# pengzhangzhi/ab_opt

Hardware: AMD Instinct MI355X
Metric: denoising steps/sec (256-res complex, 100-step sampler) (higher is better)
Workload: dtype f32

## Files before the change

ab_opt_amd/csrc/ipa_core.hip:

```cpp
#include <cstdlib>
#include <type_traits>
#include "tail_common.h"
#include "node_task.h"
#include "kernels.h"

namespace abopt {

constexpr int NPW = 8, RPW = BI / NPW;
constexpr int NTH = 1024;
constexpr int SROW = 16 * JC + 4;
constexpr int SCLD = 17;
constexpr float kLog2e = 1.4426950408889634f;
constexpr float kSqrt13 = 0.5773502691896258f;
constexpr float kScale2 = kSqrt13 * kLog2e;
constexpr float kMask2 = 1e5f * kLog2e;

__device__ __forceinline__ int sp_off(int h, int kq) { return h * JC + 4 * ((kq + (h >> 1)) & 3); }

__device__ __forceinline__ void point_local(float dx, float dy, float dz, float r0, float r1, float r2, float r3, float r4, float r5, float r6, float r7,
                                            float r8, float& lx, float& ly, float& lz, float& d, float& inv) {
    lx = __builtin_fmaf(r6, dz, __builtin_fmaf(r3, dy, r0 * dx));
    ly = __builtin_fmaf(r7, dz, __builtin_fmaf(r4, dy, r1 * dx));
    lz = __builtin_fmaf(r8, dz, __builtin_fmaf(r5, dy, r2 * dx));
    d = sqrtf(__builtin_fmaf(lz, lz, __builtin_fmaf(ly, ly, lx * lx)));
// ... 683 lines not shown

constexpr int NPW2 = 4, RPW2 = BI2 / NPW2, NTH2 = 512, HPW = 6;

#define C32_L2(x, r) __builtin_fmaf((x), kScale2, mterm_[r])
__device__ long long g_clock_probe[2];
constexpr int PROF_SLOTS = 2048;
__device__ unsigned long long g_prof_span[PROF_SLOTS][2];
__global__ void prof_span_reset_kernel() {
    const int i = blockIdx.x * 256 + threadIdx.x;
    if (i < PROF_SLOTS) { g_prof_span[i][0] = ~0ull; g_prof_span[i][1] = 0ull; }
}
struct TailArgs {
    const float *wot, *wmf, *x, *ubias, *g1, *be1, *b0, *b1, *b2, *g2, *be2;
    float* out;
    unsigned* xt;
};
template <bool NF, bool QR = false, bool QC = false> struct TailArgsT : TailArgs {};
template <> struct TailArgsT<true, false, false> : TailArgs { NodeCarryArgs nc; };
template <> struct TailArgsT<false, true, false> : TailArgs { const uint8_t* qrows; };
template <> struct TailArgsT<false, true, true> : TailArgs { const int32_t* qlist; };
struct GatherRows {
    const int32_t* ql; int64_t rowbase; int L;
    __device__ __forceinline__ int at(int il) const { const int r = il < 16 ? ql[il & 15] : -1; return (unsigned)r < (unsigned)L ? r : -1; }
    __device__ __forceinline__ int64_t load(int rl) const { return rowbase + max(at(rl), 0); }
    __device__ __forceinline__ int64_t store(int rl) const { const int r = at(rl); return r < 0 ? (int64_t)-1 : rowbase + r; }
};
constexpr int C32_LOOP_LDS_FLOATS = 3 * 32 * SROW + 2 * 32 * SCLD + 32 * SCLD + 32 * 32;
__host__ __device__ constexpr size_t core32_lds_bytes(int nchunk) { return sizeof(float) * C32_LOOP_LDS_FLOATS + (size_t)nchunk * JC; }
constexpr int C32F_PTS_OFF = ((C32_LOOP_LDS_FLOATS * 4 + 2048 + 255) / 256) * 256;
constexpr int C32F_PTSLD = H * P * 3 + 4;
constexpr int C32F_LDS_BYTES = C32F_PTS_OFF + 32 * C32F_PTSLD * 4;
constexpr int C32F_U_OFF = 0, C32F_YS_OFF = MR * XLD * 4, C32F_APA_OFF = 2 * MR * XLD * 4;
constexpr int C32F_BIAS_OFF = 2 * OT_STAGE;
static_assert(2 * OT_STAGE <= 3 * 32 * SROW * 4, "staging buffers must fit into the S/P tile");
static_assert(C32F_BIAS_OFF + 3 * F * 4 <= 3 * 32 * SROW * 4 && C32F_APA_OFF + OT_NT * AP_PLANE <= 2 * OT_STAGE && OT_NT * AP_PLANE <= 32 * C32F_PTSLD * 4, "phase-2 buffers of the fused tail");
static_assert(C32F_LDS_BYTES <= 160 * 1024, "LDS of the fused block kernel");

__device__ __forceinline__ float mul_rn(float a, float b) {
#pragma clang fp contract(off)
    return a * b;
}
__device__ __forceinline__ void stage_put4(char* buf, int row, int col, float v0, float v1, float v2, float v3) {
    unsigned h0, l0, h1, l1;
    split_pair2(v0, v1, h0, l0);
    split_pair2(v2, v3, h1, l1);
    char* d = buf + row * OT_SROW + col * 2;
    *reinterpret_cast<uint2*>(d) = make_uint2(h0, h1);
    *reinterpret_cast<uint2*>(d + OT_PLANE) = make_uint2(l0, l1);
}

constexpr int NF_CARRY_WD = 9;
static_assert(2 * H == 3 * (NTH2 / 64), "three (head, half) tasks per wave");
static_assert(MR * NF_XLDS_STRIDE * 4 <= MR * XLD * 4, "the x-term tile takes the place of the u tile");
__device__ __forceinline__ void node_carry_phase(NfLdsTerms xt, NodeCarryArgs nc, const float* __restrict__ R, const float* __restrict__ t, int L, int nchunk,
                                                           int n, int ib, int tid) {
    const int lane = tid & 63, fm = lane & 15, kq = lane >> 4;
    const int wave = __builtin_amdgcn_readfirstlane(tid >> 6);
    const int tile0 = n * nchunk + 2 * ib, tiles_end = (n + 1) * nchunk;
    const float winv = nc.w_node_frag[(int64_t)H * NF_HEAD_VEC * 4 + 1];
#pragma unroll 1
    for (int k = 0; k < 3; ++k) {
        const int h = __builtin_amdgcn_readfirstlane((wave >> 1) + 4 * k);
        const float sc = nc.spatial_coef[h];
        const float gamma = (sc > 20.f) ? sc : log1pf(expf(sc));
        const float ch_ = (-1.f * gamma * 0.16666666666666666f) / 2.f;
        const float m2c = -2.f * ch_;
        const u32x4* wg = reinterpret_cast<const u32x4*>(nc.w_node_frag) + (int64_t)h * NF_HEAD_VEC + (wave & 1) * NF_LDS_VEC;
        if (wave & 1) nf_task<1, NfX::LdsTerms, NF_CARRY_WD>(nullptr, xt, wg, R, t, nc.qfrag, nc.kvfrag, L, nchunk, tiles_end, tile0, h, ch_, m2c, winv, lane, fm, kq, nc.qk_terms, ib * BI2);
        else          nf_task<0, NfX::LdsTerms, NF_CARRY_WD>(nullptr, xt, wg, R, t, nc.qfrag, nc.kvfrag, L, nchunk, tiles_end, tile0, h, ch_, m2c, winv, lane, fm, kq, nc.qk_terms, ib * BI2);
    }
}

template <bool FUSE, bool ZT, bool NF = false, bool QROWS = false, bool QC = false>
__global__ __launch_bounds__(NTH2) void ipa_core32_kernel(const float* __restrict__ qfrag, const float* __restrict__ kvfrag, const float* __restrict__ z,
                                                          const uint8_t* __restrict__ mask, const float* __restrict__ R, const float* __restrict__ t,
                                                          float* __restrict__ feat, const float* __restrict__ pbc, int L, int nib2, int xcd_remap, int z_shared,
                                                          TailArgsT<NF, QROWS, QC> ta, int prof_slot, const float* __restrict__ zt, const float* __restrict__ zsc) {
    static_assert(FUSE || !NF, "the carried projections follow the fused tail");
    static_assert(!QROWS || (FUSE && !NF), "query rows are masked in the block nobody follows");
    static_assert(!QC || QROWS, "gathered rows are masked rows");
    constexpr int NRT = QC ? 1 : 2;
    extern __shared__ __attribute__((aligned(16))) char smem_raw[];
    float* sp = reinterpret_cast<float*>(smem_raw);
    float* scl = sp + 3 * BI2 * SROW;
    float* lsum = scl + 2 * BI2 * SCLD;
    float* mlr = lsum + BI2 * SCLD;
    uint8_t* mk = reinterpret_cast<uint8_t*>(mlr + BI2 * 32);
    int n, ib;
    {
        const int b = blockIdx.x;
        if (xcd_remap == 2) {
            const int xcd = b & 7, k = b >> 3, per = nib2 * z_shared, r = k % per;
            ib = r / z_shared; n = (xcd + 8 * (k / per)) * z_shared + r % z_shared;
        } else if (xcd_remap) { const int xcd = b & 7, k = b >> 3; n = xcd + 8 * (k / nib2); ib = k % nib2; }
        else { n = b / nib2; ib = b % nib2; }
    }
    const int tid = threadIdx.x, lane = tid & 63, fm = lane & 15, kq = lane >> 4;
    const int wave = __builtin_amdgcn_readfirstlane(tid >> 6);
    const int nchunk = (L + JC - 1) / JC, nib16 = (L + BI - 1) / BI;
    const long long probe_c0 = clock64(), probe_w0 = wall_clock64();
    if (prof_slot >= 0 && threadIdx.x == 0) atomicMin(&g_prof_span[prof_slot][0], (unsigned long long)probe_w0);
    const int i0 = ib * BI2;
    const int64_t rowbase = (int64_t)n * L;
    const int64_t zbase = z_shared ? (int64_t)(n / z_shared) * L : rowbase;
    GatherRows qg_{nullptr, rowbase, L};
    if constexpr (QC) qg_.ql = ta.qlist + ((int64_t)n * nib16 + ib) * 16;
    auto fill_mask = [&]() { for (int e = tid; e < nchunk * JC; e += NTH2) mk[e] = (e < L) ? mask[rowbase + e] : 0; };
    char* const stage = smem_raw;
    float* const ptsf = reinterpret_cast<float*>(smem_raw + C32F_PTS_OFF);
    const int64_t row0f = rowbase + i0, row_endf = rowbase + L;
    TailP2Pre<NTH2 / 64> pre;
    constexpr int RD = 12;
    struct WT { u32x4 h, l; };
    auto consumer = [&](int cb, WT (&wt)[RD]) {
        const u32x4* wfr = reinterpret_cast<const u32x4*>(ta.wot) + (int64_t)cb * OT_ST * OT_WVEC + lane;
        auto kstep = [&](int i) { return min(ot_chunk_at(min(i / OT_SPC, OT_NCH - 1)) * OT_SPC + (i % OT_SPC), OT_ST - 1); };
        f32x16 acc[4];
#pragma unroll
        for (int g = 0; g < 4; ++g) acc_zero(acc[g]);
        __syncthreads();
        const char* xrd = stage + (lane & 31) * OT_SROW + (lane >> 5) * 16;
#define C32F_KSTEP(P_, KK, NK)                                                                                           \
        {                                                                                                                \
// ... 336 lines not shown
            P2H_CHUNK(0, ch)
            if (ch + 1 < nchunk) P2H_CHUNK(1, ch + 1)
        }
        } else {
        for (; ch + 3 <= nchunk; ch += 3) { P2_CHUNK(0, ch) P2_CHUNK(1, ch + 1) P2_CHUNK(2, ch + 2) }
        if (ch < nchunk) {
            P2_CHUNK(0, ch)
            if (ch + 1 < nchunk) P2_CHUNK(1, ch + 1)
        }
        }
#undef P2H_CHUNK
#undef P2H_POS
#undef P2H_POS_LAST
#undef P2H_MF
#undef P2H_SM
#undef P2H_SPLIT
#undef P2_CHUNK
#undef P2_SLOT
#undef P2_POS
#undef P2_POS_LAST
#undef P2_MF
#undef P2_SM
#undef P2_ISSUE_Z
#undef P2_ISSUE_B
#undef P2_ZRS
#undef P2_BRS
#undef P2_RSRC
#undef P2_QNEED_FENCE
#undef P2_KOFF
#undef P2_BOFF
        if constexpr (!FUSE) {
#pragma unroll
        for (int ii = 0; ii < RPW2; ++ii) {
            const int il = il0 + ii, i = i0 + il;
            const float l_fin = mlw[ii * 32 + 1];
            if (kq == 0) lsum[il * SCLD + fm] = l_fin;
            if (i < L && fm < H) {
                const bool mi = mk[i] != 0;
                const float inv = mi ? 1.f / l_fin : 0.f;
                float* fo = feat + (rowbase + i) * FEAT + fm * C + kq * 16;
#pragma unroll
                for (int r = 0; r < 4; ++r) {
                    if constexpr (ZT) {
                        const f32x4 zs = *reinterpret_cast<const f32x4*>(zsc + (zbase + i) * C + kq * 16 + r * 4);
                        reinterpret_cast<f32x4*>(fo)[r] = (f32x4){mul_rn(accP[ii][0][r], inv * zs[0]), mul_rn(accP[ii][1][r], inv * zs[1]), mul_rn(accP[ii][2][r], inv * zs[2]), mul_rn(accP[ii][3][r], inv * zs[3])};
                    } else
                    reinterpret_cast<f32x4*>(fo)[r] = (f32x4){accP[ii][0][r] * inv, accP[ii][1][r] * inv, accP[ii][2][r] * inv, accP[ii][3][r] * inv};
                }
            }
        }
        __syncthreads();
        __syncthreads();
        } else {
#pragma unroll
        for (int ii = 0; ii < RPW2; ++ii)
            if (kq == 0) lsum[(il0 + ii) * SCLD + fm] = mlw[ii * 32 + 1];
        __syncthreads();
        float rinv[RPW2];
#pragma unroll
        for (int ii = 0; ii < RPW2; ++ii) {
            bool mi;
            if constexpr (QC) mi = qr_[ii] >= 0 && mk[max(qr_[ii], 0)] != 0;
            else { const int i = i0 + il0 + ii; mi = (i < L) && mk[min(i, L - 1)] != 0; }
            rinv[ii] = mi ? 1.f / mlw[ii * 32 + 1] : 0.f;
        }
        const int ptid = wave * 64 + lane, prow = ptid >> 3, psub = ptid & 7;
        float rr_[9], tt_[3];
        {
            int64_t grow;
            if constexpr (QC) grow = qg_.load(prow); else grow = rowbase + min(i0 + prow, L - 1);
#pragma unroll
            for (int q = 0; q < 9; ++q) rr_[q] = R[grow * 9 + q];
#pragma unroll
            for (int q = 0; q < 3; ++q) tt_[q] = t[grow * 3 + q];
        }
        __syncthreads();
        auto local_of = [&](int pt, float& lx, float& ly, float& lz, float& d, float& inv) {
            const float* a = ptsf + prow * C32F_PTSLD + pt * 3;
            point_local(a[0] - tt_[0], a[1] - tt_[1], a[2] - tt_[2], rr_[0], rr_[1], rr_[2], rr_[3], rr_[4], rr_[5], rr_[6], rr_[7], rr_[8], lx, ly, lz, d, inv);
        };
        auto put_points = [&](char* buf, int col0, int pt0, int npt, bool dir) {
            float v[24];
#pragma unroll
            for (int k = 0; k < 8; ++k) {
                if (k < npt) {
                    float lx, ly, lz, d, inv;
                    local_of(pt0 + k, lx, ly, lz, d, inv);
                    v[3 * k] = dir ? mul_rn(lx, inv) : lx; v[3 * k + 1] = dir ? mul_rn(ly, inv) : ly; v[3 * k + 2] = dir ? mul_rn(lz, inv) : lz;
                }
            }
#pragma unroll
            for (int q = 0; q < 6; ++q)
                if (4 * q < 3 * npt) stage_put4(buf, prow, col0 + 4 * q, v[4 * q], v[4 * q + 1], v[4 * q + 2], v[4 * q + 3]);
        };
#pragma unroll
        for (int p = 0; p < OT_NCH; ++p) {
            if (p >= 1 && p + 1 < OT_NCH) {
                char* buf = stage + ((p + 1) & 1) * OT_STAGE;
                const int c = ot_chunk_at(p + 1);
                if (c < 4) {
                    if (fm < H) {
#pragma unroll
                        for (int ii = 0; ii < RPW2; ++ii) {
                            if constexpr (ZT) {
                                int zr_;
                                if constexpr (QC) zr_ = max(qr_[ii], 0); else zr_ = min(i0 + il0 + ii, L - 1);
                                const f32x4 zs = *reinterpret_cast<const f32x4*>(zsc + (zbase + zr_) * C + kq * 16 + c * 4);
                                stage_put4(buf, il0 + ii, fm * 16 + kq * 4, mul_rn(accP[ii][0][c], rinv[ii] * zs[0]), mul_rn(accP[ii][1][c], rinv[ii] * zs[1]),
                                           mul_rn(accP[ii][2][c], rinv[ii] * zs[2]), mul_rn(accP[ii][3][c], rinv[ii] * zs[3]));
                            } else
                            stage_put4(buf, il0 + ii, fm * 16 + kq * 4, mul_rn(accP[ii][0][c], rinv[ii]), mul_rn(accP[ii][1][c], rinv[ii]),
                                       mul_rn(accP[ii][2][c], rinv[ii]), mul_rn(accP[ii][3][c], rinv[ii]));
                        }
                    }
                } else if (c == 6) {
                    put_points(buf, psub * 24, psub * 8, 8, false);
                } else if (c == 7) {
                    put_points(buf, psub * 12, 64 + psub * 4, 4, false);
                    float dd[12];
#pragma unroll
                    for (int k = 0; k < 12; ++k) { float lx, ly, lz, inv; local_of(psub * 12 + k, lx, ly, lz, dd[k], inv); }
#pragma unroll
                    for (int q = 0; q < 3; ++q) stage_put4(buf, prow, 96 + psub * 12 + 4 * q, dd[4 * q], dd[4 * q + 1], dd[4 * q + 2], dd[4 * q + 3]);
                } else if (c == 8) {
                    put_points(buf, psub * 24, psub * 8, 8, true);
                } else {
                    put_points(buf, psub * 12, 64 + psub * 4, 4, true);
                }
            }
            __syncthreads();
        }
        }
    } else if (wave < NPW2 + 2) {
        const int h0 = (wave - NPW2) * HPW;
        const f32x4* kvn = reinterpret_cast<const f32x4*>(kvfrag) + (int64_t)n * nchunk * H * 512;
        f32x4 qr[HPW][NRT][4];
        const int qrow_ = QC ? max(qg_.at(fm), 0) : 0;
#pragma unroll
        for (int hh = 0; hh < HPW; ++hh)
#pragma unroll
            for (int rt = 0; rt < NRT; ++rt) {
                const f32x4* qg;
                if constexpr (QC) qg = reinterpret_cast<const f32x4*>(qfrag) + (((int64_t)n * nib16 + (qrow_ >> 4)) * H + h0 + hh) * (4 * 64) + kq * 16 + (qrow_ & 15);
                else qg = reinterpret_cast<const f32x4*>(qfrag) + (((int64_t)n * nib16 + min(2 * ib + rt, nib16 - 1)) * H + h0 + hh) * (4 * 64) + lane;
#pragma unroll
                for (int s_ = 0; s_ < 4; ++s_) qr[hh][rt][s_] = qg[s_ * 64];
            }
        f32x4 kf[2][4];
#define A2_ISSUE(B, HH, CH) { const f32x4* fr_ = kvn + ((int64_t)min((CH), nchunk - 1) * H + h0 + (HH)) * 512 + lane;   \
        _Pragma("unroll") for (int s_ = 0; s_ < 4; ++s_) kf[B][s_] = fr_[s_ * 64]; }
        auto produce = [&](int c, int buf) {
#pragma unroll
            for (int hh = 0; hh < HPW; ++hh) {
                const int h = h0 + hh;
                if (hh + 1 < HPW) { if (hh & 1) A2_ISSUE(0, hh + 1, c) else A2_ISSUE(1, hh + 1, c) } else A2_ISSUE(0, 0, c + 1)
#pragma unroll
                for (int rt = 0; rt < NRT; ++rt) {
                    const f32x4 q0 = qr[hh][rt][0], q1 = qr[hh][rt][1], q2 = qr[hh][rt][2], q3 = qr[hh][rt][3];
                    f32x4 acc0 = (f32x4){0.f, 0.f, 0.f, 0.f}, acc1 = acc0;
                    if constexpr (ZT) {
                        const u32x4 kh = __builtin_bit_cast(u32x4, kf[hh & 1][0]), kl = __builtin_bit_cast(u32x4, kf[hh & 1][1]);
                        const u32x4 qh = __builtin_bit_cast(u32x4, q0), ql = __builtin_bit_cast(u32x4, q1);
                        acc0 = mfma_h(kl, qh, acc0); acc0 = mfma_h(kh, ql, acc0);
#pragma unroll
                        for (int s = 0; s < 4; ++s) { acc1 = mfma4(kf[hh & 1][2][s], q2[s], acc1); if (s == 1) acc0 = mfma_h(kh, qh, acc0); }
#pragma unroll
                        for (int s = 0; s < 3; ++s) acc1 = mfma4(kf[hh & 1][3][s], q3[s], acc1);
                    }
                    else {
#pragma unroll
                    for (int s = 0; s < 4; ++s) { acc0 = mfma4(kf[hh & 1][0][s], q0[s], acc0); acc1 = mfma4(kf[hh & 1][2][s], q2[s], acc1); }
#pragma unroll
                    for (int s = 0; s < 4; ++s) { acc0 = mfma4(kf[hh & 1][1][s], q1[s], acc0); if (s < 3) acc1 = mfma4(kf[hh & 1][3][s], q3[s], acc1); }
                    }
                    const f32x4 sres = acc0 + acc1;
                    *reinterpret_cast<f32x4*>(sp + (buf * BI2 + rt * 16 + fm) * SROW + sp_off(h, kq)) = sres;
                }
                __builtin_amdgcn_sched_barrier(0);
            }
        };
        A2_ISSUE(0, 0, 0)
        fill_mask();
        __syncthreads();
        produce(0, 0);
        __syncthreads();
        int buf = 1;
        for (int c = 1; c < nchunk; ++c) {
            produce(c, buf);
            buf = (buf == 2) ? 0 : buf + 1;
            __syncthreads();
        }
        __syncthreads();
        if constexpr (!FUSE) {
        __syncthreads();
        __syncthreads();
        } else {
        WT raw[RD];
        consumer_prefetch(wave - NPW2, raw);
        __syncthreads();
        tail_p2_stage_bias(reinterpret_cast<float (*)[F]>(smem_raw + C32F_BIAS_OFF), ta.b0, ta.b1, ta.b2, tid - NPW2 * 64);
        consumer(wave - NPW2, raw);
        }
#undef A2_ISSUE
    } else {
        const int h0 = (wave - NPW2 - 2) * HPW;
        const f32x4* kvn = reinterpret_cast<const f32x4*>(kvfrag) + (int64_t)n * nchunk * H * 512;
        f32x4 vf[2][4];
        f32x4 accV[HPW][2][2], accT[HPW][2][2];
#pragma unroll
        for (int hh = 0; hh < HPW; ++hh)
#pragma unroll
            for (int rt = 0; rt < 2; ++rt)
#pragma unroll
                for (int k = 0; k < 2; ++k) { accV[hh][rt][k] = (f32x4){0.f, 0.f, 0.f, 0.f}; accT[hh][rt][k] = (f32x4){0.f, 0.f, 0.f, 0.f}; }
#define C2_ISSUE(B, HH, CH) { const f32x4* fr_ = kvn + ((int64_t)min((CH), nchunk - 1) * H + h0 + (HH)) * 512 + 4 * 64 + lane; \
        _Pragma("unroll") for (int s_ = 0; s_ < 4; ++s_) vf[B][s_] = fr_[s_ * 64]; }
        auto consume = [&](int c, int buf) {
            const int par = c & 1;
#pragma unroll
            for (int hh = 0; hh < HPW; ++hh) {
                const int h = h0 + hh;
                if (hh + 1 < HPW) { if (hh & 1) C2_ISSUE(0, hh + 1, c) else C2_ISSUE(1, hh + 1, c) } else C2_ISSUE(0, 0, c + 1)
#pragma unroll
                for (int rt = 0; rt < NRT; ++rt) {
                    const float sc = scl[(par * BI2 + rt * 16 + fm) * SCLD + h];
                    const f32x4 pa = *reinterpret_cast<const f32x4*>(sp + (buf * BI2 + rt * 16 + fm) * SROW + sp_off(h, kq));
                    if (!(FUSE && __builtin_amdgcn_ballot_w64(sc != 1.f) == 0ull)) { accV[hh][rt][0] *= sc; accV[hh][rt][1] *= sc; accT[hh][rt][0] *= sc; accT[hh][rt][1] *= sc; }
#pragma unroll
                    for (int s = 0; s < 4; ++s) {
                        accV[hh][rt][0] = mfma4(vf[hh & 1][s][0], pa[s], accV[hh][rt][0]);
                        accV[hh][rt][1] = mfma4(vf[hh & 1][s][1], pa[s], accV[hh][rt][1]);
                        accT[hh][rt][0] = mfma4(vf[hh & 1][s][2], pa[s], accT[hh][rt][0]);
                        accT[hh][rt][1] = mfma4(vf[hh & 1][s][3], pa[s], accT[hh][rt][1]);
                    }
                }
                __builtin_amdgcn_sched_barrier(0);
            }
        };
        C2_ISSUE(0, 0, 0)
        fill_mask();
        __syncthreads();
        __syncthreads();
        __syncthreads();
        int buf = 0;
        for (int c = 1; c < nchunk; ++c) {
            consume(c - 1, buf);
            buf = (buf == 2) ? 0 : buf + 1;
            __syncthreads();
        }
        consume(nchunk - 1, buf);
        WT raw[RD];
        __syncthreads();
        float* pts = FUSE ? ptsf : sp;
        char* nbuf = stage + (wave - NPW2 - 2) * OT_STAGE;
#pragma unroll
        for (int hh = 0; hh < HPW; ++hh) {
            const int h = h0 + hh;
#pragma unroll
            for (int rt = 0; rt < 2; ++rt) {
                const int il = rt * 16 + fm, i = i0 + il;
                bool mi;
                if constexpr (QC) { const int qi = rt == 0 ? qg_.at(fm) : -1; mi = qi >= 0 && mk[max(qi, 0)] != 0; }
                else mi = (i < L) && mk[min(i, L - 1)] != 0;
                const float inv = mi ? 1.f / lsum[il * SCLD + h] : 0.f;
                if constexpr (FUSE) {
                    const f32x4 a0 = accV[hh][rt][0], a1 = accV[hh][rt][1];
                    stage_put4(nbuf, il, hh * D + kq * 4, mul_rn(a0[0], inv), mul_rn(a0[1], inv), mul_rn(a0[2], inv), mul_rn(a0[3], inv));
                    stage_put4(nbuf, il, hh * D + 16 + kq * 4, mul_rn(a1[0], inv), mul_rn(a1[1], inv), mul_rn(a1[2], inv), mul_rn(a1[3], inv));
                } else if (i < L) {
                    float* fo = feat + (rowbase + i) * FEAT + H * C + h * D + kq * 4;
                    *reinterpret_cast<f32x4*>(fo) = accV[hh][rt][0] * inv;
                    *reinterpret_cast<f32x4*>(fo + 16) = accV[hh][rt][1] * inv;
                }
                float* po = pts + il * (FUSE ? C32F_PTSLD : H * P * 3) + h * (P * 3) + kq * 3;
#pragma unroll
                for (int r = 0; r < 3; ++r) { po[r] = accT[hh][rt][0][r] * inv; po[12 + r] = accT[hh][rt][1][r] * inv; }
            }
        }
        if constexpr (FUSE) {
            consumer_prefetch(wave - NPW2, raw);
            consumer(wave - NPW2, raw);
        }
        else __syncthreads();
#undef C2_ISSUE
    }
    if constexpr (!FUSE) {
        persist_point_epilogue(sp, R, t, feat, rowbase, i0, L, tid, NTH2, BI2);
    } else {
        const int64_t row0 = row0f, row_end = row_endf;
        if constexpr (QC) pre = tail_p2_prefetch<NTH2 / 64>(ta.x, ta.ubias, mask, ta.g1, ta.be1, ta.wmf, row0, row_end, wave, lane, qg_);
        else pre = tail_p2_prefetch<NTH2 / 64>(ta.x, ta.ubias, mask, ta.g1, ta.be1, ta.wmf, row0, row_end, wave, lane);
        float (*bias)[F] = reinterpret_cast<float (*)[F]>(smem_raw + C32F_BIAS_OFF);
        __syncthreads();
        const float (*us)[XLD] = reinterpret_cast<const float (*)[XLD]>(smem_raw + C32F_U_OFF);
        auto get_u = [&](int rl) { return *reinterpret_cast<const float2*>(&us[rl][2 * lane]); };
        if constexpr (QC)
        tail_p2_run<NTH2 / 64, false>(pre, get_u, reinterpret_cast<float (*)[XLD]>(smem_raw + C32F_YS_OFF), bias, smem_raw + C32F_APA_OFF,
                                      smem_raw + C32F_PTS_OFF, ta.wmf, ta.g2, ta.be2, ta.out, nullptr, 0, row0, row_end, wave, lane, ta.xt, nullptr, 0, qg_);
        else
        tail_p2_run<NTH2 / 64, false>(pre, get_u, reinterpret_cast<float (*)[XLD]>(smem_raw + C32F_YS_OFF), bias, smem_raw + C32F_APA_OFF,
                                      smem_raw + C32F_PTS_OFF, ta.wmf, ta.g2, ta.be2, ta.out, nullptr, 0, row0, row_end, wave, lane, ta.xt,
                                      NF ? reinterpret_cast<unsigned*>(smem_raw + C32F_U_OFF) : nullptr, NF_XLDS_STRIDE);
        if constexpr (NF) {
            __syncthreads();
            node_carry_phase((NfLdsTerms)(smem_raw + C32F_U_OFF), ta.nc, R, t, L, nchunk, n, ib, tid);
        }
    }
    if (blockIdx.x == 0 && tid == 0) { g_clock_probe[0] = clock64() - probe_c0; g_clock_probe[1] = wall_clock64() - probe_w0; }
    if (prof_slot >= 0 && tid == 0) atomicMax(&g_prof_span[prof_slot][1], (unsigned long long)wall_clock64());
}

struct WbList { const float* w[8]; };

__global__ __launch_bounds__(256) void pair_bias_cache_kernel(const float* __restrict__ z, WbList wl, int num_layers, float* __restrict__ cache,
                                                              int64_t rows, int L, int nchunk) {
    __shared__ __attribute__((aligned(16))) float zst[4][JC][ZSLD];
    const int wave = threadIdx.x >> 6, lane = threadIdx.x & 63, fm = lane & 15, kq = lane >> 4;
    const int64_t unit = (int64_t)blockIdx.x * 4 + wave;
    if (unit >= rows * 4) return;
    const int64_t row = unit >> 2;
    const int q0 = (int)(unit & 3);
    if (q0 >= nchunk) return;
    const float* zi = z + (row * (int64_t)L) * C;
    f32x4 wv[6][4];
#pragma unroll
    for (int l = 0; l < 6; ++l)
#pragma unroll
        for (int q = 0; q < 4; ++q) wv[l][q] = (l < num_layers && fm < H) ? reinterpret_cast<const f32x4*>(wl.w[l] + fm * C + kq * 16)[q] : (f32x4){0.f, 0.f, 0.f, 0.f};
    f32x4 zn[4];
#pragma unroll
    for (int r = 0; r < 4; ++r) zn[r] = *(reinterpret_cast<const f32x4*>(zi + (int64_t)min(q0 * JC + kq * 4 + r, L - 1) * C) + fm);
    for (int ch = q0; ch < nchunk; ch += 4) {
        wave_lds_sync();
#pragma unroll
        for (int r = 0; r < 4; ++r) *reinterpret_cast<f32x4*>(&zst[wave][kq * 4 + r][fm * 4]) = zn[r];
        if (ch + 4 < nchunk) {
#pragma unroll
            for (int r = 0; r < 4; ++r) zn[r] = *(reinterpret_cast<const f32x4*>(zi + (int64_t)min((ch + 4) * JC + kq * 4 + r, L - 1) * C) + fm);
        }
        wave_lds_sync();
        f32x4 za[4];
#pragma unroll
        for (int q = 0; q < 4; ++q) za[q] = *reinterpret_cast<const f32x4*>(&zst[wave][fm][kq * 16 + q * 4]);
        const int64_t u = (int64_t)ch * rows + row;
        auto layer = [&](int l, const f32x4 (&w4)[4]) {
            f32x4 acc4[4];
#pragma unroll
            for (int q = 0; q < 4; ++q) {
                acc4[q] = mfma4(za[q][0], w4[q][0], (f32x4){0.f, 0.f, 0.f, 0.f});
                acc4[q] = mfma4(za[q][1], w4[q][1], acc4[q]); acc4[q] = mfma4(za[q][2], w4[q][2], acc4[q]); acc4[q] = mfma4(za[q][3], w4[q][3], acc4[q]);
            }
            const f32x4 acc = (acc4[0] + acc4[1]) + (acc4[2] + acc4[3]);
            if (fm < H) *reinterpret_cast<f32x4*>(cache + ((int64_t)l * rows * nchunk + u) * (H * JC) + fm * JC + kq * 4) = acc;
        };
#pragma unroll
        for (int l = 0; l < 6; ++l)
            if (l < num_layers) layer(l, wv[l]);
        for (int l = 6; l < num_layers; ++l) {
// ... 275 lines not shown
```

ab_opt_amd/csrc/node_task.h:

```cpp
#pragma once
#include "ipa_common.h"

namespace abopt {

constexpr int NF_F = 128;
constexpr int NF_TILES = 12, NF_HT = NF_TILES / 2, NF_WAVES = 4;
constexpr int NF_KS = NF_F / 32, NF_SPL = 2;
constexpr int NF_HEAD_VEC = NF_TILES * NF_KS * NF_SPL * 64;
constexpr int NF_LDS_VEC = NF_HEAD_VEC / 2;

__device__ __forceinline__ float quad_bcast0(float v) { return __uint_as_float(__builtin_amdgcn_update_dpp(0u, __float_as_uint(v), 0x00, 0xf, 0xf, false)); }
__device__ __forceinline__ float quad_bcast1(float v) { return __uint_as_float(__builtin_amdgcn_update_dpp(0u, __float_as_uint(v), 0x55, 0xf, 0xf, false)); }
__device__ __forceinline__ float quad_bcast2(float v) { return __uint_as_float(__builtin_amdgcn_update_dpp(0u, __float_as_uint(v), 0xAA, 0xf, 0xf, false)); }

enum class NfX { GlobalF32, GlobalTerms, LdsTerms };
constexpr int NF_XLDS_STRIDE = NF_F + 4;
typedef const __attribute__((address_space(3))) unsigned* NfLdsTerms;
typedef const __attribute__((address_space(3))) u32x4* NfLdsVec;
__device__ __forceinline__ float nf_mul_rn(float a, float b) {
#pragma clang fp contract(off)
    return a * b;
}
template <int HALF, NfX XS, int WD, class XP, class WP>
__device__ __forceinline__ void nf_task(const float* __restrict__ x, XP xt, WP wl, const float* __restrict__ R, const float* __restrict__ t,
                                        float* __restrict__ qfrag, float* __restrict__ kvfrag, int L, int nchunk, int total_tiles, int tile0, int h,
                                        float ch_, float m2c, float winv, int lane, int fm, int kq, int qk_terms, int xrow0 = 0) {
    constexpr bool XT = XS != NfX::GlobalF32;
    constexpr int XLD_ = XS == NfX::LdsTerms ? NF_XLDS_STRIDE : NF_F;
    int64_t rowbase[2], row[2];
    int cbs[2];
#pragma unroll
    for (int rt = 0; rt < 2; ++rt) {
        const int tile = min(tile0 + rt, total_tiles - 1);
        const int n = tile / nchunk;
        cbs[rt] = tile % nchunk;
        rowbase[rt] = (int64_t)n * L;
        row[rt] = rowbase[rt] + min(cbs[rt] * JC + fm, L - 1);
    }
    auto xvec = [&](int rt, int word) {
        if constexpr (XS == NfX::LdsTerms) return *reinterpret_cast<NfLdsVec>(xt + (min(cbs[rt] * JC + fm, L - 1) - xrow0) * XLD_ + word);
        else return *reinterpret_cast<const u32x4*>(xt + row[rt] * XLD_ + word);
    };
    f32x4 xa[2][2];
    Split2 xn[2];
#pragma unroll
    for (int rt = 0; rt < 2; ++rt) {
        if constexpr (XT) {
            xn[rt].h = xvec(rt, kq * 4);
            xn[rt].l = xvec(rt, 64 + kq * 4);
        } else {
            xa[rt][0] = *reinterpret_cast<const f32x4*>(x + row[rt] * NF_F + kq * 8);
            xa[rt][1] = *reinterpret_cast<const f32x4*>(x + row[rt] * NF_F + kq * 8 + 4);
        }
    }
    f32x4 acc[2][NF_HT];
#pragma unroll
    for (int rt = 0; rt < 2; ++rt)
#pragma unroll
        for (int T = 0; T < NF_HT; ++T) acc[rt][T] = (f32x4){0.f, 0.f, 0.f, 0.f};
    const auto wh = wl + lane;
    static_assert(WD >= 2 && WD <= NF_KS * NF_HT, "weight ring");
    u32x4 wa[WD][NF_SPL];
    auto wfrag_at = [&](int g_, int sp) { return wh[(((g_ % NF_HT) * NF_KS + g_ / NF_HT) * NF_SPL + sp) * 64]; };
#pragma unroll
    for (int g = 0; g < WD - 1; ++g)
#pragma unroll
        for (int sp = 0; sp < NF_SPL; ++sp) wa[g][sp] = wfrag_at(g, sp);
    Split2 xs[2];
#pragma unroll
    for (int g = 0; g < NF_KS * NF_HT; ++g) {
        const int s = g / NF_HT, T = g % NF_HT;
        if (T == 0) {
#pragma unroll
            for (int rt = 0; rt < 2; ++rt) {
                if constexpr (XT) xs[rt] = xn[rt];
                else xs[rt] = split2(xa[rt][0], xa[rt][1]);
            }
            if (s + 1 < NF_KS) {
#pragma unroll
                for (int rt = 0; rt < 2; ++rt) {
                    if constexpr (XT) {
                        xn[rt].h = xvec(rt, (s + 1) * 16 + kq * 4);
                        xn[rt].l = xvec(rt, 64 + (s + 1) * 16 + kq * 4);
                    } else {
                        xa[rt][0] = *reinterpret_cast<const f32x4*>(x + row[rt] * NF_F + (s + 1) * 32 + kq * 8);
                        xa[rt][1] = *reinterpret_cast<const f32x4*>(x + row[rt] * NF_F + (s + 1) * 32 + kq * 8 + 4);
                    }
                }
            }
        }
        if (g + WD - 1 < NF_KS * NF_HT) {
#pragma unroll
            for (int sp = 0; sp < NF_SPL; ++sp) wa[(g + WD - 1) % WD][sp] = wfrag_at(g + WD - 1, sp);
        }
        const u32x4 wH = wa[g % WD][0], wL = wa[g % WD][1];
        const bool swap = (HALF == 1) && (T >= 2);
#define NF_PROD(XT, WT)                                                                                                         \
        if (swap) { acc[0][T] = mfma_h(xs[0].XT, WT, acc[0][T]); acc[1][T] = mfma_h(xs[1].XT, WT, acc[1][T]); }               \
        else      { acc[0][T] = mfma_h(WT, xs[0].XT, acc[0][T]); acc[1][T] = mfma_h(WT, xs[1].XT, acc[1][T]); }
        NF_PROD(l, wH) NF_PROD(h, wL) NF_PROD(h, wH)
#undef NF_PROD
        __builtin_amdgcn_sched_barrier(0);
    }
    auto sq = [](const f32x4& g) { return fmaf(g[2], g[2], fmaf(g[1], g[1], g[0] * g[0])); };
#pragma unroll
    for (int rt = 0; rt < 2; ++rt) {
        if (tile0 + rt >= total_tiles) break;
        const int tile = tile0 + rt;
#pragma unroll
        for (int T = 0; T < NF_HT; ++T) acc[rt][T] *= winv;
        float Rm[9], tv[3];
#pragma unroll
        for (int k = 0; k < 9; ++k) Rm[k] = R[row[rt] * 9 + k];
#pragma unroll
        for (int k = 0; k < 3; ++k) tv[k] = t[row[rt] * 3 + k];
        auto dot3 = [](float a, float b, float c, float d, float e, float f, float t_) { return fmaf(e, f, fmaf(a, b, nf_mul_rn(c, d))) + t_; };
        auto to_global = [&](const f32x4& p) {
            return (f32x4){dot3(Rm[0], p[0], Rm[1], p[1], Rm[2], p[2], tv[0]), dot3(Rm[3], p[0], Rm[4], p[1], Rm[5], p[2], tv[1]),
                           dot3(Rm[6], p[0], Rm[7], p[1], Rm[8], p[2], tv[2]), 0.f};
        };
        f32x4* outq = reinterpret_cast<f32x4*>(qfrag) + ((int64_t)tile * H + h) * (4 * 64) + lane;
        f32x4* outk = reinterpret_cast<f32x4*>(kvfrag) + ((int64_t)tile * H + h) * (8 * 64) + lane;
        if (HALF == 0) {
            const float s = 0.17677669529663687f;
            if (qk_terms) {
                const f32x4 q0 = (f32x4){nf_mul_rn(acc[rt][0][0], s), nf_mul_rn(acc[rt][0][1], s), nf_mul_rn(acc[rt][0][2], s), nf_mul_rn(acc[rt][0][3], s)};
                const f32x4 q1 = (f32x4){nf_mul_rn(acc[rt][1][0], s), nf_mul_rn(acc[rt][1][1], s), nf_mul_rn(acc[rt][1][2], s), nf_mul_rn(acc[rt][1][3], s)};
                Split2 tq;
#pragma unroll
                for (int p = 0; p < 2; ++p) {
                    unsigned hw, lw;
                    split_pair2(q0[2 * p], q0[2 * p + 1], hw, lw);
                    tq.h[p] = hw; tq.l[p] = lw;
                    hw = pk_f16(q1[2 * p], q1[2 * p + 1]);
                    tq.h[2 + p] = hw;
                    tq.l[2 + p] = pk_f16(fmaf(acc[rt][1][2 * p], s, -f16lo_f32(hw)), fmaf(acc[rt][1][2 * p + 1], s, -f16hi_f32(hw)));
                }
                const Split2 tk = split2(acc[rt][2], acc[rt][3]);
                outq[0] = __builtin_bit_cast(f32x4, tq.h); outq[64] = __builtin_bit_cast(f32x4, tq.l);
                outk[0] = __builtin_bit_cast(f32x4, tk.h); outk[64] = __builtin_bit_cast(f32x4, tk.l);
            } else {
            outq[0] = acc[rt][0] * s; outq[64] = acc[rt][1] * s;
            outk[0] = acc[rt][2]; outk[64] = acc[rt][3];
            }
            f32x4 ga = to_global(acc[rt][4]), gb = to_global(acc[rt][5]);
            const float nq = rows_sum(sq(ga) + sq(gb));
            ga *= m2c; gb *= m2c;
            ga[3] = kq == 0 ? ch_ * nq : (kq == 1 ? ch_ : 0.f);
            gb[3] = 0.f;
            outq[128] = ga; outq[192] = gb;
        } else {
            f32x4 ga = to_global(acc[rt][0]), gb = to_global(acc[rt][1]);
            const float nk = rows_sum(sq(ga) + sq(gb));
            ga[3] = kq == 0 ? 1.f : (kq == 1 ? nk : 0.f);
            outk[128] = ga; outk[192] = gb;
            const int c = fm & 3, cr = min(c, 2);
#pragma unroll
            for (int r = 0; r < 4; ++r) {
                const int64_t rr = rowbase[rt] + min(cbs[rt] * JC + kq * 4 + r, L - 1);
                const float r0 = R[rr * 9 + cr * 3], r1 = R[rr * 9 + cr * 3 + 1], r2 = R[rr * 9 + cr * 3 + 2], r3 = t[rr * 3 + cr];
                const float xa_ = quad_bcast0(acc[rt][4][r]), ya = quad_bcast1(acc[rt][4][r]), za = quad_bcast2(acc[rt][4][r]);
                const float xb = quad_bcast0(acc[rt][5][r]), yb = quad_bcast1(acc[rt][5][r]), zb = quad_bcast2(acc[rt][5][r]);
                float g0 = dot3(r0, xa_, r1, ya, r2, za, r3);
                float g1 = dot3(r0, xb, r1, yb, r2, zb, r3);
                if (c == 3) { g0 = 0.f; g1 = 0.f; }
                outk[(4 + r) * 64] = (f32x4){acc[rt][2][r], acc[rt][3][r], g0, g1};
            }
        }
    }
}

}
```

Before: 31140.

## Prefetch node-carry weights, zsc scales and K/V fragments; stage frames in LDS

Splits the node-carry task into main and epilogue stages. The next head's weight ring and spatial coefficient are now prefetched before the current epilogue runs, and the first ring fill is issued before the barrier. The rotation frames R/t are written once into LDS, so the epilogue reads them from shared memory instead of global memory. The output-staging loop prefetches the next chunk's zsc scale vectors, and in the gathered-row (QC) variant every head's K/V fragments get their own register slot and are issued one chunk ahead. The cost is higher register pressure and more scheduling complexity.

Measured after the change: 31340, median of 6. Within noise of the previous version (+0.6%).

```diff
diff --git a/ab_opt_amd/csrc/ipa_core.hip b/ab_opt_amd/csrc/ipa_core.hip
--- a/ab_opt_amd/csrc/ipa_core.hip
+++ b/ab_opt_amd/csrc/ipa_core.hip
@@ -759,23 +759,45 @@
 constexpr int NF_CARRY_WD = 9;
 static_assert(2 * H == 3 * (NTH2 / 64), "three (head, half) tasks per wave");
 static_assert(MR * NF_XLDS_STRIDE * 4 <= MR * XLD * 4, "the x-term tile takes the place of the u tile");
-__device__ __forceinline__ void node_carry_phase(NfLdsTerms xt, NodeCarryArgs nc, const float* __restrict__ R, const float* __restrict__ t, int L, int nchunk,
-                                                           int n, int ib, int tid) {
-    const int lane = tid & 63, fm = lane & 15, kq = lane >> 4;
-    const int wave = __builtin_amdgcn_readfirstlane(tid >> 6);
+static_assert(BI2 == 2 * JC, "a workgroup's rows are exactly the two row tiles of its tasks: every clamped row of a task lies in the frame tile");
+struct NodeCarryPre { NfRing<NF_CARRY_WD> ring; float sc, winv; };
+__device__ __forceinline__ const u32x4* node_carry_weights(const NodeCarryArgs& nc, int wave, int lane, int k) {
+    const int h = __builtin_amdgcn_readfirstlane((wave >> 1) + 4 * k);
+    return reinterpret_cast<const u32x4*>(nc.w_node_frag) + (int64_t)h * NF_HEAD_VEC + (wave & 1) * NF_LDS_VEC + lane;
+}
+__device__ __forceinline__ void node_carry_request(const NodeCarryArgs& nc, int tid, NodeCarryPre& pre) {
+    const int lane = tid & 63, wave = __builtin_amdgcn_readfirstlane(tid >> 6);
+    pre.sc = nc.spatial_coef[__builtin_amdgcn_readfirstlane(wave >> 1)];
+    pre.winv = nc.w_node_frag[(int64_t)H * NF_HEAD_VEC * 4 + 1];
+    nf_ring_fill(pre.ring, node_carry_weights(nc, wave, lane, 0));
+}
+template <int HALF>
+__device__ __forceinline__ void node_carry_tasks(NfLdsTerms xt, NfFramesLds fr, const NodeCarryArgs& nc, NodeCarryPre& pre, int L, int nchunk, int n, int ib, int wave,
+                                                 int lane) {
+    const int fm = lane & 15, kq = lane >> 4;
     const int tile0 = n * nchunk + 2 * ib, tiles_end = (n + 1) * nchunk;
-    const float winv = nc.w_node_frag[(int64_t)H * NF_HEAD_VEC * 4 + 1];
+    const NfRows rows = nf_rows(L, nchunk, tiles_end, tile0, fm);
+    float sc = pre.sc;
 #pragma unroll 1
     for (int k = 0; k < 3; ++k) {
         const int h = __builtin_amdgcn_readfirstlane((wave >> 1) + 4 * k);
-        const float sc = nc.spatial_coef[h];
+        f32x4 acc[2][NF_HT];
+        nf_main<HALF, NfX::LdsTerms, NF_CARRY_WD, false>(nullptr, xt, node_carry_weights(nc, wave, lane, k), rows, pre.ring, acc, L, fm, kq, ib * BI2);
+        const int kn = min(k + 1, 2);
+        const float sc_next = nc.spatial_coef[__builtin_amdgcn_readfirstlane((wave >> 1) + 4 * kn)];
+        nf_ring_fill(pre.ring, node_carry_weights(nc, wave, lane, kn));
+        __builtin_amdgcn_sched_barrier(0);
         const float gamma = (sc > 20.f) ? sc : log1pf(expf(sc));
         const float ch_ = (-1.f * gamma * 0.16666666666666666f) / 2.f;
         const float m2c = -2.f * ch_;
-        const u32x4* wg = reinterpret_cast<const u32x4*>(nc.w_node_frag) + (int64_t)h * NF_HEAD_VEC + (wave & 1) * NF_LDS_VEC;
-        if (wave & 1) nf_task<1, NfX::LdsTerms, NF_CARRY_WD>(nullptr, xt, wg, R, t, nc.qfrag, nc.kvfrag, L, nchunk, tiles_end, tile0, h, ch_, m2c, winv, lane, fm, kq, nc.qk_terms, ib * BI2);
-        else          nf_task<0, NfX::LdsTerms, NF_CARRY_WD>(nullptr, xt, wg, R, t, nc.qfrag, nc.kvfrag, L, nchunk, tiles_end, tile0, h, ch_, m2c, winv, lane, fm, kq, nc.qk_terms, ib * BI2);
-    }
+        nf_epilogue<HALF>(acc, rows, fr, nullptr, nullptr, nc.qfrag, nc.kvfrag, L, tiles_end, tile0, h, ch_, m2c, pre.winv, lane, fm, kq, nc.qk_terms);
+        sc = sc_next;
+    }
+}
+__device__ __forceinline__ void node_carry_phase(NfLdsTerms xt, NfFramesLds fr, const NodeCarryArgs& nc, NodeCarryPre& pre, int L, int nchunk, int n, int ib, int tid) {
+    const int lane = tid & 63, wave = __builtin_amdgcn_readfirstlane(tid >> 6);
+    if (wave & 1) node_carry_tasks<1>(xt, fr, nc, pre, L, nchunk, n, ib, wave, lane);
+    else          node_carry_tasks<0>(xt, fr, nc, pre, L, nchunk, n, ib, wave, lane);
 }
 
 template <bool FUSE, bool ZT, bool NF = false, bool QROWS = false, bool QC = false>
@@ -1218,6 +1240,16 @@
         __syncthreads();
         __syncthreads();
         } else {
+        f32x4 zsn_[RPW2];
+        auto zsc_request = [&](int c) {
+#pragma unroll
+            for (int ii = 0; ii < RPW2; ++ii) {
+                int zr_;
+                if constexpr (QC) zr_ = max(qr_[ii], 0); else zr_ = min(i0 + il0 + ii, L - 1);
+                zsn_[ii] = *reinterpret_cast<const f32x4*>(zsc + (zbase + zr_) * C + kq * 16 + c * 4);
+            }
+        };
+        if constexpr (ZT) zsc_request(0);
 #pragma unroll
         for (int ii = 0; ii < RPW2; ++ii)
             if (kq == 0) lsum[(il0 + ii) * SCLD + fm] = mlw[ii * 32 + 1];
@@ -1241,6 +1273,14 @@
             for (int q = 0; q < 3; ++q) tt_[q] = t[grow * 3 + q];
         }
         __syncthreads();
+        if constexpr (NF) {
+            if (psub == 0) {
+#pragma unroll
+                for (int q = 0; q < 9; ++q) mlr[prow * NF_FRLD + q] = rr_[q];
+#pragma unroll
+                for (int q = 0; q < 3; ++q) mlr[prow * NF_FRLD + 9 + q] = tt_[q];
+            }
+        }
         auto local_of = [&](int pt, float& lx, float& ly, float& lz, float& d, float& inv) {
             const float* a = ptsf + prow * C32F_PTSLD + pt * 3;
             point_local(a[0] - tt_[0], a[1] - tt_[1], a[2] - tt_[2], rr_[0], rr_[1], rr_[2], rr_[3], rr_[4], rr_[5], rr_[6], rr_[7], rr_[8], lx, ly, lz, d, inv);
@@ -1265,13 +1305,17 @@
                 char* buf = stage + ((p + 1) & 1) * OT_STAGE;
                 const int c = ot_chunk_at(p + 1);
                 if (c < 4) {
+                    f32x4 zsc_[RPW2];
+                    if constexpr (ZT) {
+#pragma unroll
+                        for (int ii = 0; ii < RPW2; ++ii) zsc_[ii] = zsn_[ii];
+                        if (c + 1 < 4) zsc_request(c + 1);
+                    }
                     if (fm < H) {
 #pragma unroll
                         for (int ii = 0; ii < RPW2; ++ii) {
                             if constexpr (ZT) {
-                                int zr_;
-                                if constexpr (QC) zr_ = max(qr_[ii], 0); else zr_ = min(i0 + il0 + ii, L - 1);
-                                const f32x4 zs = *reinterpret_cast<const f32x4*>(zsc + (zbase + zr_) * C + kq * 16 + c * 4);
+                                const f32x4 zs = zsc_[ii];
                                 stage_put4(buf, il0 + ii, fm * 16 + kq * 4, mul_rn(accP[ii][0][c], rinv[ii] * zs[0]), mul_rn(accP[ii][1][c], rinv[ii] * zs[1]),
                                            mul_rn(accP[ii][2][c], rinv[ii] * zs[2]), mul_rn(accP[ii][3][c], rinv[ii] * zs[3]));
                             } else
@@ -1312,40 +1356,45 @@
 #pragma unroll
                 for (int s_ = 0; s_ < 4; ++s_) qr[hh][rt][s_] = qg[s_ * 64];
             }
-        f32x4 kf[2][4];
+        constexpr int KRD = QC ? HPW : 2;
+        f32x4 kf[KRD][4];
 #define A2_ISSUE(B, HH, CH) { const f32x4* fr_ = kvn + ((int64_t)min((CH), nchunk - 1) * H + h0 + (HH)) * 512 + lane;   \
         _Pragma("unroll") for (int s_ = 0; s_ < 4; ++s_) kf[B][s_] = fr_[s_ * 64]; }
         auto produce = [&](int c, int buf) {
 #pragma unroll
             for (int hh = 0; hh < HPW; ++hh) {
                 const int h = h0 + hh;
-                if (hh + 1 < HPW) { if (hh & 1) A2_ISSUE(0, hh + 1, c) else A2_ISSUE(1, hh + 1, c) } else A2_ISSUE(0, 0, c + 1)
+                if constexpr (!QC) { if (hh + 1 < HPW) { if (hh & 1) A2_ISSUE(0, hh + 1, c) else A2_ISSUE(1, hh + 1, c) } else A2_ISSUE(0, 0, c + 1) }
 #pragma unroll
                 for (int rt = 0; rt < NRT; ++rt) {
                     const f32x4 q0 = qr[hh][rt][0], q1 = qr[hh][rt][1], q2 = qr[hh][rt][2], q3 = qr[hh][rt][3];
                     f32x4 acc0 = (f32x4){0.f, 0.f, 0.f, 0.f}, acc1 = acc0;
                     if constexpr (ZT) {
-                        const u32x4 kh = __builtin_bit_cast(u32x4, kf[hh & 1][0]), kl = __builtin_bit_cast(u32x4, kf[hh & 1][1]);
+                        const u32x4 kh = __builtin_bit_cast(u32x4, kf[hh % KRD][0]), kl = __builtin_bit_cast(u32x4, kf[hh % KRD][1]);
                         const u32x4 qh = __builtin_bit_cast(u32x4, q0), ql = __builtin_bit_cast(u32x4, q1);
                         acc0 = mfma_h(kl, qh, acc0); acc0 = mfma_h(kh, ql, acc0);
 #pragma unroll
-                        for (int s = 0; s < 4; ++s) { acc1 = mfma4(kf[hh & 1][2][s], q2[s], acc1); if (s == 1) acc0 = mfma_h(kh, qh, acc0); }
-#pragma unroll
-                        for (int s = 0; s < 3; ++s) acc1 = mfma4(kf[hh & 1][3][s], q3[s], acc1);
+                        for (int s = 0; s < 4; ++s) { acc1 = mfma4(kf[hh % KRD][2][s], q2[s], acc1); if (s == 1) acc0 = mfma_h(kh, qh, acc0); }
+#pragma unroll
+                        for (int s = 0; s < 3; ++s) acc1 = mfma4(kf[hh % KRD][3][s], q3[s], acc1);
                     }
                     else {
 #pragma unroll
-                    for (int s = 0; s < 4; ++s) { acc0 = mfma4(kf[hh & 1][0][s], q0[s], acc0); acc1 = mfma4(kf[hh & 1][2][s], q2[s], acc1); }
-#pragma unroll
-                    for (int s = 0; s < 4; ++s) { acc0 = mfma4(kf[hh & 1][1][s], q1[s], acc0); if (s < 3) acc1 = mfma4(kf[hh & 1][3][s], q3[s], acc1); }
+                    for (int s = 0; s < 4; ++s) { acc0 = mfma4(kf[hh % KRD][0][s], q0[s], acc0); acc1 = mfma4(kf[hh % KRD][2][s], q2[s], acc1); }
+#pragma unroll
+                    for (int s = 0; s < 4; ++s) { acc0 = mfma4(kf[hh % KRD][1][s], q1[s], acc0); if (s < 3) acc1 = mfma4(kf[hh % KRD][3][s], q3[s], acc1); }
                     }
                     const f32x4 sres = acc0 + acc1;
                     *reinterpret_cast<f32x4*>(sp + (buf * BI2 + rt * 16 + fm) * SROW + sp_off(h, kq)) = sres;
                 }
+                if constexpr (QC) A2_ISSUE(hh, hh, c + 1)
                 __builtin_amdgcn_sched_barrier(0);
             }
         };
-        A2_ISSUE(0, 0, 0)
+        if constexpr (QC) {
+#pragma unroll
+            for (int hh = 0; hh < HPW; ++hh) A2_ISSUE(hh, hh, 0)
+        } else A2_ISSUE(0, 0, 0)
         fill_mask();
         __syncthreads();
         produce(0, 0);
@@ -1371,7 +1420,8 @@
     } else {
         const int h0 = (wave - NPW2 - 2) * HPW;
         const f32x4* kvn = reinterpret_cast<const f32x4*>(kvfrag) + (int64_t)n * nchunk * H * 512;
-        f32x4 vf[2][4];
+        constexpr int VRD = QC ? HPW : 2;
+        f32x4 vf[VRD][4];
         f32x4 accV[HPW][2][2], accT[HPW][2][2];
 #pragma unroll
         for (int hh = 0; hh < HPW; ++hh)
@@ -1386,7 +1436,7 @@
 #pragma unroll
             for (int hh = 0; hh < HPW; ++hh) {
                 const int h = h0 + hh;
-                if (hh + 1 < HPW) { if (hh & 1) C2_ISSUE(0, hh + 1, c) else C2_ISSUE(1, hh + 1, c) } else C2_ISSUE(0, 0, c + 1)
+                if constexpr (!QC) { if (hh + 1 < HPW) { if (hh & 1) C2_ISSUE(0, hh + 1, c) else C2_ISSUE(1, hh + 1, c) } else C2_ISSUE(0, 0, c + 1) }
 #pragma unroll
                 for (int rt = 0; rt < NRT; ++rt) {
                     const float sc = scl[(par * BI2 + rt * 16 + fm) * SCLD + h];
@@ -1394,16 +1444,20 @@
                     if (!(FUSE && __builtin_amdgcn_ballot_w64(sc != 1.f) == 0ull)) { accV[hh][rt][0] *= sc; accV[hh][rt][1] *= sc; accT[hh][rt][0] *= sc; accT[hh][rt][1] *= sc; }
 #pragma unroll
                     for (int s = 0; s < 4; ++s) {
-                        accV[hh][rt][0] = mfma4(vf[hh & 1][s][0], pa[s], accV[hh][rt][0]);
-                        accV[hh][rt][1] = mfma4(vf[hh & 1][s][1], pa[s], accV[hh][rt][1]);
-                        accT[hh][rt][0] = mfma4(vf[hh & 1][s][2], pa[s], accT[hh][rt][0]);
-                        accT[hh][rt][1] = mfma4(vf[hh & 1][s][3], pa[s], accT[hh][rt][1]);
+                        accV[hh][rt][0] = mfma4(vf[hh % VRD][s][0], pa[s], accV[hh][rt][0]);
+                        accV[hh][rt][1] = mfma4(vf[hh % VRD][s][1], pa[s], accV[hh][rt][1]);
+                        accT[hh][rt][0] = mfma4(vf[hh % VRD][s][2], pa[s], accT[hh][rt][0]);
+                        accT[hh][rt][1] = mfma4(vf[hh % VRD][s][3], pa[s], accT[hh][rt][1]);
                     }
                 }
+                if constexpr (QC) C2_ISSUE(hh, hh, c + 1)
                 __builtin_amdgcn_sched_barrier(0);
             }
         };
-        C2_ISSUE(0, 0, 0)
+        if constexpr (QC) {
+#pragma unroll
+            for (int hh = 0; hh < HPW; ++hh) C2_ISSUE(hh, hh, 0)
+        } else C2_ISSUE(0, 0, 0)
         fill_mask();
         __syncthreads();
         __syncthreads();
@@ -1468,8 +1522,10 @@
                                       smem_raw + C32F_PTS_OFF, ta.wmf, ta.g2, ta.be2, ta.out, nullptr, 0, row0, row_end, wave, lane, ta.xt,
                                       NF ? reinterpret_cast<unsigned*>(smem_raw + C32F_U_OFF) : nullptr, NF_XLDS_STRIDE);
         if constexpr (NF) {
+            NodeCarryPre ncp;
+            node_carry_request(ta.nc, tid, ncp);
             __syncthreads();
-            node_carry_phase((NfLdsTerms)(smem_raw + C32F_U_OFF), ta.nc, R, t, L, nchunk, n, ib, tid);
+            node_carry_phase((NfLdsTerms)(smem_raw + C32F_U_OFF), NfFramesLds{(const __attribute__((address_space(3))) float*)mlr, i0}, ta.nc, ncp, L, nchunk, n, ib, tid);
         }
     }
     if (blockIdx.x == 0 && tid == 0) { g_clock_probe[0] = clock64() - probe_c0; g_clock_probe[1] = wall_clock64() - probe_w0; }
diff --git a/ab_opt_amd/csrc/node_task.h b/ab_opt_amd/csrc/node_task.h
--- a/ab_opt_amd/csrc/node_task.h
+++ b/ab_opt_amd/csrc/node_task.h
@@ -21,22 +21,48 @@
 #pragma clang fp contract(off)
     return a * b;
 }
-template <int HALF, NfX XS, int WD, class XP, class WP>
-__device__ __forceinline__ void nf_task(const float* __restrict__ x, XP xt, WP wl, const float* __restrict__ R, const float* __restrict__ t,
-                                        float* __restrict__ qfrag, float* __restrict__ kvfrag, int L, int nchunk, int total_tiles, int tile0, int h,
-                                        float ch_, float m2c, float winv, int lane, int fm, int kq, int qk_terms, int xrow0 = 0) {
-    constexpr bool XT = XS != NfX::GlobalF32;
-    constexpr int XLD_ = XS == NfX::LdsTerms ? NF_XLDS_STRIDE : NF_F;
-    int64_t rowbase[2], row[2];
-    int cbs[2];
+struct NfFramesGlobal {
+    __device__ __forceinline__ float Rk(const float* __restrict__ R, int64_t grow, int, int k) const { return R[grow * 9 + k]; }
+    __device__ __forceinline__ float tk(const float* __restrict__ t, int64_t grow, int, int k) const { return t[grow * 3 + k]; }
+};
+constexpr int NF_FRLD = 13;
+struct NfFramesLds {
+    const __attribute__((address_space(3))) float* tile;
+    int row0;
+    __device__ __forceinline__ float Rk(const float*, int64_t, int rs, int k) const { return tile[(rs - row0) * NF_FRLD + k]; }
+    __device__ __forceinline__ float tk(const float*, int64_t, int rs, int k) const { return tile[(rs - row0) * NF_FRLD + 9 + k]; }
+};
+struct NfRows { int64_t rowbase[2], row[2]; int cbs[2]; };
+__device__ __forceinline__ NfRows nf_rows(int L, int nchunk, int total_tiles, int tile0, int fm) {
+    NfRows r;
 #pragma unroll
     for (int rt = 0; rt < 2; ++rt) {
         const int tile = min(tile0 + rt, total_tiles - 1);
         const int n = tile / nchunk;
-        cbs[rt] = tile % nchunk;
-        rowbase[rt] = (int64_t)n * L;
-        row[rt] = rowbase[rt] + min(cbs[rt] * JC + fm, L - 1);
-    }
+        r.cbs[rt] = tile % nchunk;
+        r.rowbase[rt] = (int64_t)n * L;
+        r.row[rt] = r.rowbase[rt] + min(r.cbs[rt] * JC + fm, L - 1);
+    }
+    return r;
+}
+template <int WD> struct NfRing { u32x4 wa[WD][NF_SPL]; };
+template <class WP> __device__ __forceinline__ auto nf_wfrag_at(WP wh, int g_, int sp) { return wh[(((g_ % NF_HT) * NF_KS + g_ / NF_HT) * NF_SPL + sp) * 64]; }
+template <int WD, class WP>
+__device__ __forceinline__ void nf_ring_fill(NfRing<WD>& ring, WP wh) {
+    static_assert(WD >= 2 && WD <= NF_KS * NF_HT, "weight ring");
+#pragma unroll
+    for (int g = 0; g < WD - 1; ++g)
+#pragma unroll
+        for (int sp = 0; sp < NF_SPL; ++sp) ring.wa[g][sp] = nf_wfrag_at(wh, g, sp);
+}
+template <int HALF, NfX XS, int WD, bool COLD, class XP, class WP>
+__device__ __forceinline__ void nf_main(const float* __restrict__ x, XP xt, WP wh, const NfRows& rows, NfRing<WD>& ring, f32x4 (&acc)[2][NF_HT], int L, int fm, int kq,
+                                        int xrow0) {
+    constexpr bool XT = XS != NfX::GlobalF32;
+    constexpr int XLD_ = XS == NfX::LdsTerms ? NF_XLDS_STRIDE : NF_F;
+    const int64_t (&row)[2] = rows.row;
+    const int (&cbs)[2] = rows.cbs;
+    u32x4 (&wa)[WD][NF_SPL] = ring.wa;
     auto xvec = [&](int rt, int word) {
         if constexpr (XS == NfX::LdsTerms) return *reinterpret_cast<NfLdsVec>(xt + (min(cbs[rt] * JC + fm, L - 1) - xrow0) * XLD_ + word);
         else return *reinterpret_cast<const u32x4*>(xt + row[rt] * XLD_ + word);
@@ -53,19 +79,11 @@
             xa[rt][1] = *reinterpret_cast<const f32x4*>(x + row[rt] * NF_F + kq * 8 + 4);
         }
     }
-    f32x4 acc[2][NF_HT];
 #pragma unroll
     for (int rt = 0; rt < 2; ++rt)
 #pragma unroll
         for (int T = 0; T < NF_HT; ++T) acc[rt][T] = (f32x4){0.f, 0.f, 0.f, 0.f};
-    const auto wh = wl + lane;
-    static_assert(WD >= 2 && WD <= NF_KS * NF_HT, "weight ring");
-    u32x4 wa[WD][NF_SPL];
-    auto wfrag_at = [&](int g_, int sp) { return wh[(((g_ % NF_HT) * NF_KS + g_ / NF_HT) * NF_SPL + sp) * 64]; };
-#pragma unroll
-    for (int g = 0; g < WD - 1; ++g)
-#pragma unroll
-        for (int sp = 0; sp < NF_SPL; ++sp) wa[g][sp] = wfrag_at(g, sp);
+    if constexpr (COLD) nf_ring_fill(ring, wh);
     Split2 xs[2];
 #pragma unroll
     for (int g = 0; g < NF_KS * NF_HT; ++g) {
@@ -91,7 +109,7 @@
         }
         if (g + WD - 1 < NF_KS * NF_HT) {
 #pragma unroll
-            for (int sp = 0; sp < NF_SPL; ++sp) wa[(g + WD - 1) % WD][sp] = wfrag_at(g + WD - 1, sp);
+            for (int sp = 0; sp < NF_SPL; ++sp) wa[(g + WD - 1) % WD][sp] = nf_wfrag_at(wh, g + WD - 1, sp);
         }
         const u32x4 wH = wa[g % WD][0], wL = wa[g % WD][1];
         const bool swap = (HALF == 1) && (T >= 2);
@@ -102,6 +120,12 @@
 #undef NF_PROD
         __builtin_amdgcn_sched_barrier(0);
     }
+}
+template <int HALF, class FR>
+__device__ __forceinline__ void nf_epilogue(f32x4 (&acc)[2][NF_HT], const NfRows& rows, FR fr, const float* __restrict__ R, const float* __restrict__ t, float* __restrict__ qfrag, float* __restrict__ kvfrag, int L,
+                                            int total_tiles, int tile0, int h, float ch_, float m2c, float winv, int lane, int fm, int kq, int qk_terms) {
+    const int64_t (&rowbase)[2] = rows.rowbase;
+    const int (&cbs)[2] = rows.cbs;
     auto sq = [](const f32x4& g) { return fmaf(g[2], g[2], fmaf(g[1], g[1], g[0] * g[0])); };
 #pragma unroll
     for (int rt = 0; rt < 2; ++rt) {
@@ -111,9 +135,9 @@
         for (int T = 0; T < NF_HT; ++T) acc[rt][T] *= winv;
         float Rm[9], tv[3];
 #pragma unroll
-        for (int k = 0; k < 9; ++k) Rm[k] = R[row[rt] * 9 + k];
-#pragma unroll
-        for (int k = 0; k < 3; ++k) tv[k] = t[row[rt] * 3 + k];
+        for (int k = 0; k < 9; ++k) Rm[k] = fr.Rk(R, rows.row[rt], min(cbs[rt] * JC + fm, L - 1), k);
+#pragma unroll
+        for (int k = 0; k < 3; ++k) tv[k] = fr.tk(t, rows.row[rt], min(cbs[rt] * JC + fm, L - 1), k);
         auto dot3 = [](float a, float b, float c, float d, float e, float f, float t_) { return fmaf(e, f, fmaf(a, b, nf_mul_rn(c, d))) + t_; };
         auto to_global = [&](const f32x4& p) {
             return (f32x4){dot3(Rm[0], p[0], Rm[1], p[1], Rm[2], p[2], tv[0]), dot3(Rm[3], p[0], Rm[4], p[1], Rm[5], p[2], tv[1]),
@@ -157,8 +181,9 @@
             const int c = fm & 3, cr = min(c, 2);
 #pragma unroll
             for (int r = 0; r < 4; ++r) {
-                const int64_t rr = rowbase[rt] + min(cbs[rt] * JC + kq * 4 + r, L - 1);
-                const float r0 = R[rr * 9 + cr * 3], r1 = R[rr * 9 + cr * 3 + 1], r2 = R[rr * 9 + cr * 3 + 2], r3 = t[rr * 3 + cr];
+                const int rs = min(cbs[rt] * JC + kq * 4 + r, L - 1);
+                const int64_t rr = rowbase[rt] + rs;
+                const float r0 = fr.Rk(R, rr, rs, cr * 3), r1 = fr.Rk(R, rr, rs, cr * 3 + 1), r2 = fr.Rk(R, rr, rs, cr * 3 + 2), r3 = fr.tk(t, rr, rs, cr);
                 const float xa_ = quad_bcast0(acc[rt][4][r]), ya = quad_bcast1(acc[rt][4][r]), za = quad_bcast2(acc[rt][4][r]);
                 const float xb = quad_bcast0(acc[rt][5][r]), yb = quad_bcast1(acc[rt][5][r]), zb = quad_bcast2(acc[rt][5][r]);
                 float g0 = dot3(r0, xa_, r1, ya, r2, za, r3);
@@ -169,5 +194,16 @@
         }
     }
 }
-
-}
+template <int HALF, NfX XS, int WD, class XP, class WP>
+__device__ __forceinline__ void nf_task(const float* __restrict__ x, XP xt, WP wl, const float* __restrict__ R, const float* __restrict__ t,
+                                        float* __restrict__ qfrag, float* __restrict__ kvfrag, int L, int nchunk, int total_tiles, int tile0, int h,
+                                        float ch_, float m2c, float winv, int lane, int fm, int kq, int qk_terms, int xrow0 = 0) {
+    const NfRows rows = nf_rows(L, nchunk, total_tiles, tile0, fm);
+    const auto wh = wl + lane;
+    NfRing<WD> ring;
+    f32x4 acc[2][NF_HT];
+    nf_main<HALF, XS, WD, true>(x, xt, wh, rows, ring, acc, L, fm, kq, xrow0);
+    nf_epilogue<HALF>(acc, rows, NfFramesGlobal{}, R, t, qfrag, kvfrag, L, total_tiles, tile0, h, ch_, m2c, winv, lane, fm, kq, qk_terms);
+}
+
+}
```
